# msyriac/orphics

Hardware: AMD Instinct MI355X
Metric: QE kappa reconstructions/sec on 8192^2 maps (higher is better)
Workload: dtype f64

## Files before the change

### orphics_amd/csrc/fft.hip

```cpp
#include <cmath>
#include <vector>
#include "fft_launch.hpp"
#include "fft_r2c_w64.hpp"
#include "fft_r2c_rs4096.hpp"
#include "fft_divbin.hpp"

namespace oa {

template <typename T, int MODE, class SEQ>
__global__ __launch_bounds__(row_maxnt<SEQ>(), waves_per_eu<T>()) void row_fft_kernel(RowArgs<T> a) {
    GpuCtx c{oa_dyn_smem};
    row_fft_body<T, MODE, SEQ>(c, a);
}

#ifndef OA_W64_OCC
#define OA_W64_OCC 1
#endif
__global__ __launch_bounds__(64, OA_W64_OCC) void row_r2c_w64_kernel(RowW64Args a) {
    GpuCtx c{oa_dyn_smem};
    row_r2c_w64_body(c, a);
}

template <typename T, class SEQ, int LR, bool PF>
__global__ __launch_bounds__(row_maxnt<SEQ>(), (sizeof(T) == 8 || PF ? 2 : 3)) void row_r2c_rsplit_kernel(RowArgs<T> a) {
// ... 28 lines not shown
    row_r2c_rs_body<T, 13, 3, PF>(c, a);
}

template <typename T, class SEQF, int LR, int LOGC>
__global__ __launch_bounds__((sizeof(T) == 8 ? 512 : 1024)) void col_fband_pack_kernel(ColFBandArgs<T> a, cx<T>* out) {
    GpuCtx c{nullptr};
    col_fband_pack_body<T, SEQF, LR, LOGC>(c, a, out);
}
template <typename T, class SEQF, int LR, int LOGC>
__global__ __launch_bounds__((sizeof(T) == 8 ? 512 : 1024), (sizeof(T) == 8 ? 2 : 4)) void col_fband_kernel(ColFBandArgs<T> a) {
    GpuCtx c{oa_dyn_smem};
    col_fband_body<T, SEQF, LR, LOGC>(c, a);
}

template <typename T, class SEQF, int LOGC>
__global__ __launch_bounds__((sizeof(T) == 8 ? 512 : 1024)) void col_fband3_pack_kernel(ColFBandArgs<T> a, cx<T>* out) {
    GpuCtx c{nullptr};
    col_fband3_pack_body<T, SEQF, LOGC>(c, a, out);
}
template <typename T, class SEQF, int LOGC>
__global__ __launch_bounds__((sizeof(T) == 8 ? 512 : 1024), (sizeof(T) == 8 ? 2 : 4)) void col_fband3_kernel(ColFBandArgs<T> a) {
    GpuCtx c{oa_dyn_smem};
    col_fband3_body<T, SEQF, LOGC>(c, a);
}

__global__ __launch_bounds__(128, 1) void row_r2c_w64x2_kernel(RowW64Args a) {
    GpuCtx c{oa_dyn_smem};
    row_r2c_w64x2_body(c, a);
}

#ifndef OA_QE_WAVES_PER_EU
#define OA_QE_WAVES_PER_EU 3
#endif
template <typename T, class SEQ> constexpr int qe_waves_per_eu() {
    return sizeof(T) == 8 ? 1 : (row_maxnt<SEQ>() > 256 ? 2 : OA_QE_WAVES_PER_EU);
}

template <typename T, class SEQ, int NZ>
__global__ __launch_bounds__(row_maxnt<SEQ>(), (qe_waves_per_eu<T, SEQ>())) void row_qe_kernel(RowQeArgs<T> a) {
    GpuCtx c{oa_dyn_smem};
#ifdef OA_QE_INPLACE
    row_qe_body_inplace<T, SEQ>(c, a);
#else
    row_qe_body<T, SEQ, NZ>(c, a);
#endif
}
// ... 260 lines not shown
            if (e != hipSuccess) rc = fail(std::string("fft launch: ") + hipGetErrorString(e));
        });
        if (!ok) rc = fail("fft: unsupported R-split column stage");
    }
    template <typename T>
    void col_fband3(int gx, int gz, size_t smem, int logMy, const ColFBandArgs<T>& a) {
        if (rc) return;
        constexpr int nt = sizeof(T) == 4 ? 1024 : 512, lc11 = sizeof(T) == 4 ? 3 : 2;
        if (logMy == 11) go(col_fband3_kernel<T, Seq<16, 16, 8>, lc11>, dim3(gx, 4, gz), nt, smem, a);
        else if (logMy == 10) go(col_fband3_kernel<T, Seq<16, 8, 8>, lc11 + 1>, dim3(gx, 4, gz), nt, smem, a);
        else rc = fail("fft: unsupported 3 x 2^k R-split column stage");
    }
    template <typename T>
    void col_fband3_pack(int gx, int logMy, const ColFBandArgs<T>& a, cx<T>* out) {
        if (rc) return;
        constexpr int nt = sizeof(T) == 4 ? 1024 : 512, lc11 = sizeof(T) == 4 ? 3 : 2;
        if (logMy == 11) hipLaunchKernelGGL((col_fband3_pack_kernel<T, Seq<16, 16, 8>, lc11>), dim3(gx, 4), dim3(nt), 0, st, a, out);
        else if (logMy == 10) hipLaunchKernelGGL((col_fband3_pack_kernel<T, Seq<16, 8, 8>, lc11 + 1>), dim3(gx, 4), dim3(nt), 0, st, a, out);
        else { rc = fail("fft: unsupported 3 x 2^k R-split column stage"); return; }
        const hipError_t e = hipGetLastError();
        if (e != hipSuccess) rc = fail(std::string("fft launch: ") + hipGetErrorString(e));
    }
    template <typename T>
    void row_qe(int grid, int nt, size_t smem, const RowQeArgs<T>& a) {
        const bool ok = dispatch_seq_qe(a.logL, [&](auto seq) {
            using S = decltype(seq);
            if constexpr (seq_logl<S>() >= 4) {
                if (nt > row_maxnt<S>()) { if (!rc) rc = fail("fft: row workgroup size exceeds its launch bound"); return; }
                if constexpr (S::n >= 2 && sizeof(T) == 4) {
                    dispatch_nz<S>(qe_first_stage_nz(a.logL, S::rget(0), a.win), [&](auto nzc) {
                        go(row_qe_kernel<T, S, decltype(nzc)::value>, dim3(grid), nt, smem, a);
                    });
                } else {
                    go(row_qe_kernel<T, S, 0>, dim3(grid), nt, smem, a);
                }
            } else {
                if (!rc) rc = fail("fft: unsupported row length");
            }
        });
        if (!ok && !rc) rc = fail("fft: unsupported row length");
    }
    template <typename T>
    void row_qe_pair8(int pairs, int M, const RowQeArgs<T>& a) {
        const bool ok = dispatch_rq8(M, a.win, a.lr, a.chain != nullptr, [&](auto ac, auto nzc, auto lay, auto ch) {
            constexpr int A = decltype(ac)::value;
            if (ch.value && !a.tab) { if (!rc) rc = fail("fft: estimator chains need a table"); return; }
// ... 748 lines not shown
```

### orphics_amd/csrc/fft_fband.hpp

```cpp
#pragma once
#include "fft_kernels.hpp"
#include "fft_mixed.hpp"
#ifndef FB_STAMP
#define FB_STAMP(i)
#endif

namespace oa {

template <typename T>
struct ColFBandArgs {
    const cx<T>* in;
    long kplane, pitch;
    const T* FG; const T* FH;
    long fpitch;
    const cx<T>* fgh;
    const T* lxd; const T* lyd;
    cx<T>* gx; cx<T>* gy; cx<T>* h;
    long opitch;
    int width;
    const cx<T>* tw;
    int ny_full, rband;
    long in_moff, out_moff;
    const cx<T>* tw3 = nullptr;
};
// ... 276 lines not shown
    const FBand3Store<T> st{outp + zmap * a.out_moff + (long)k1 * a.opitch + c0, (unsigned)(R * a.opitch), leg < 3 ? ncols : 0, ti, q};
    fft_pipeline<T, false, false, true, SI>(ctx, s + sid * (Q << LOGC), tq, NTS, logQ, LOGC, 0, twq, logQ, NoLoad{}, st);
    FB_STAMP(5);
}

template <typename T, class SEQF, int LOGC, class Ctx>
OA_HD void col_fband3_pack_body(Ctx& ctx, const ColFBandArgs<T>& a, cx<T>* out) {
    constexpr int logL = seq_total_log<SEQF>(), R = 4, Q = 1 << (logL - 4), C = 1 << LOGC;
    constexpr int NT = (1 << (logL + LOGC)) / EPT;
    const int tid = ctx.tid(), tile = ctx.bid_x(), k1 = ctx.bid_y(), c0 = tile << LOGC;
    const int c = tid & (C - 1), m = tid >> LOGC;
    cx<T>* o = out + (((long)k1 * ctx.grid_x() + tile) * 3) * NT + tid;
#pragma unroll
    for (int e = 0; e < 3; ++e) {
        const int yf = k1 + R * fband3_bin<Q>(m, e);
        bool live = c0 + c < a.width;
        if (a.rband) live = live && !(yf >= a.rband && yf <= a.ny_full - a.rband);
        cx<T> f = mk<T>((T)0, (T)0);
        if (live) { const long fi = (long)yf * a.fpitch + (c0 + c); f = mk<T>(a.FG[fi], a.FH[fi]); }
        o[e * NT] = f;
    }
}

}
```

### orphics_amd/csrc/fft_plan.hpp

```cpp
#pragma once
#include <cmath>
#include <cstdlib>
#include <vector>
#include "fft_kernels.hpp"
#include "fft_fband.hpp"
#include "fft_rowqe8.hpp"

namespace oa {

template <typename T>
inline std::vector<cx<T>> make_twiddles(int M) {
    std::vector<cx<T>> t((size_t)M);
    const long double tau = 6.283185307179586476925286766559005768L;
    for (int k = 0; k < M; ++k) {
        long double a = tau * (long double)k / (long double)M;
        t[(size_t)k].x = (T)cosl(a);
        t[(size_t)k].y = (T)(-sinl(a));
    }
    return t;
}

inline long kpitch_for(int nx) { return nx / 2 + 16; }

inline bool is_pow2(int v) { return v > 0 && (v & (v - 1)) == 0; }
inline bool is_m3(int v) { return v >= 3 && v % 3 == 0 && is_pow2(v / 3); }
// ... 75 lines not shown
        static const int narrow = [] { const char* e = exp_env("OA_FBAND_NARROW"); return e ? atoi(e) : 0; }();
        return (sizeof(T) == 4 ? 14 : 13) - (narrow > 0 ? 1 : 0);
    }
    template <class Launcher>
    void legs_fband(Launcher& q, const Fft2dPlan<T>& cv, const cx<T>* Y, long kplane, long pin, const T* FG, const T* FH, const T* lxd,
                    const T* lyd, cx<T>* gx, cx<T>* gy, cx<T>* h, int wmax, int rband, long pout, int nmaps = 1, long in_moff = 0,
                    long out_moff = 0, const cx<T>* fgh = nullptr, cx<T>* pack_out = nullptr) const {
        ColFBandArgs<T> a{};
        a.in = Y; a.kplane = kplane; a.pitch = pin; a.FG = FG; a.FH = FH; a.fpitch = kp; a.lxd = lxd; a.lyd = lyd; a.fgh = fgh;
        a.gx = gx; a.gy = gy; a.h = h; a.opitch = pout; a.width = clampw(wmax); a.tw = cv.tw_y; a.ny_full = ny; a.rband = clampr(rband);
        a.in_moff = in_moff; a.out_moff = out_moff;
        const int lt = fband_lt(), lc = lt - cv.logNy, Cs = 1 << lc;
        const int logMq = cv.logNy - (logNy - cv.logNy);
        const size_t smem = ((size_t)(1 << lt) + tw_lds_size(cv.logNy) + tw_lds_size(logMq) + (logNy - cv.logNy == 1 ? 0 : (1 << logMq))) * sizeof(cx<T>);
        if (pack_out) q.col_fband_pack((a.width + Cs - 1) / Cs, 1 << (logNy - cv.logNy), cv.logNy, a, pack_out);
        else q.col_fband((a.width + Cs - 1) / Cs, 1 << (logNy - cv.logNy), nmaps, smem, cv.logNy, a);
    }
    static bool has_rsplit3(int logNy, int logNx, int my3, int wl) {
        if (!is_m3(my3)) return false;
        const int myf = m3_pow2(my3);
        return (myf == 1024 || myf == 2048) && logNy - ilog2(myf) == 2 && has_rsplit(logNy, logNx, myf, wl) && fband_lt() == (sizeof(T) == 4 ? 14 : 13) &&
               div_lt() == fband_lt();
    }
    template <class Launcher>
    void legs_fband3(Launcher& q, const Fft2dPlan<T>& cv, const cx<T>* twf, const cx<T>* Y, long kplane, long pin, const T* FG, const T* FH,
                     const T* lxd, const T* lyd, cx<T>* gx, cx<T>* gy, cx<T>* h, int wmax, int rband, long pout, int nmaps = 1, long in_moff = 0,
                     long out_moff = 0, const cx<T>* fgh = nullptr, cx<T>* pack_out = nullptr) const {
        ColFBandArgs<T> a{};
        a.in = Y; a.kplane = kplane; a.pitch = pin; a.FG = FG; a.FH = FH; a.fpitch = kp; a.lxd = lxd; a.lyd = lyd; a.fgh = fgh;
        a.gx = gx; a.gy = gy; a.h = h; a.opitch = pout; a.width = clampw(wmax); a.tw = twf; a.tw3 = cv.tw_y; a.ny_full = ny; a.rband = clampr(rband);
        a.in_moff = in_moff; a.out_moff = out_moff;
        const int logMy = logNy - 2, lt = fband_lt(), lc = lt - logMy, Cs = 1 << lc, logQ = logMy - 4;
        const size_t smem = ((size_t)(1 << lt) + tw_lds_size(logMy) + tw_lds_size(logQ) + 3 * (1 << logQ)) * sizeof(cx<T>);
        if (pack_out) q.col_fband3_pack((a.width + Cs - 1) / Cs, logMy, a, pack_out);
        else q.col_fband3((a.width + Cs - 1) / Cs, nmaps, smem, logMy, a);
    }
    long fband_table_entries(const Fft2dPlan<T>& cv, int wmax) const {
        const int lc = fband_lt() - cv.logNy, Cs = 1 << lc;
        return (long)((clampw(wmax) + Cs - 1) / Cs) * Cs * cv.ny;
    }
    long fband3_table_entries(const Fft2dPlan<T>& cv, int wmax) const {
        const int lc = fband_lt() - (logNy - 2), Cs = 1 << lc;
        return (long)((clampw(wmax) + Cs - 1) / Cs) * Cs * cv.ny;
    }

    double row_grid_scale(int mrow) const { return (mrow > 0 && mrow < nx) ? (double)nx / (double)mrow : 1.0; }
    bool rows_qe_is_pair(int win, int wout, int mrow) const {
        if (mrow <= 0 || ny % 2) return false;
        const int M = mrow < nx ? mrow : nx;
        if (rq8_is_m3(M)) return rq8_ready(M) && rq8_covers(M, win, wout);
        return is_pow2(M) && M >= 1024 && M <= 8192 && 2L * win + wout <= M;
    }
    bool rows_qe_lr1(int win, int wout, int mrow) const { return mrow == 4096 && mrow <= nx && rq8_ready(mrow) && rq8_covers(mrow, win, wout); }
    static bool& rowqe8_on() {
        static bool on = exp_env("OA_NO_ROWQE8") == nullptr;
// ... 309 lines not shown
```

### orphics_amd/csrc/pipeline.hip

```cpp
#include <dlfcn.h>
#include <cstdlib>
#include <algorithm>
#include <string>
#include <utility>
#include <vector>
#include "common.hpp"
#include "fft_plan.hpp"

namespace oa {

constexpr int MC_BATCH_MAX = 6;

struct Pipeline {
    const void* FG = nullptr; const void* FH = nullptr; const void* Fn = nullptr;
    int wl = 0, wk = 0, rl = 0, rk = 0, mrow = -1;
    int mcol = -1;
    int my = 0;
    int my3 = 0;
    int map_grid() const { return my3 ? my3 : my; }
    void* work = nullptr;
    void* c[3] = {nullptr, nullptr, nullptr};
    void* g[2] = {nullptr, nullptr};
    void* kT = nullptr;
    void* kk = nullptr;
// ... 162 lines not shown
    q->my3 = 0;
    const bool want3 = q->mcol > 0 && is_m3(q->mcol);
    const long need = std::max(2L * q->rl + q->rk, 2L * q->rk);
    if (want3 && q->rl > 0 && q->rk > 0 && q->mcol < need)
        return fail("column grid < max(2*leg_rows + kappa_rows, 2*kappa_rows) would alias the leg products into the kept rows");
    if (int rc = resolve_my(p, q->mcol, q->rl, q->rk, &q->my)) return rc;
    const int my3 = want3 ? q->mcol : (q->mcol < 0 && q->my > 0 && q->my % 4 == 0 ? q->my / 4 * 3 : 0);
    bool ok = my3 > 0 && q->my == m3_pow2(my3) && my3 >= need && qe_rsplit_lr(p, q->my, q->wl, q->wk, q->mrow) == 2;
    if (ok) {
        if (int rc = plan_ensure_col_grid(p, my3)) return rc;
        ok = qe_rsplit_lr(p, my3, q->wl, q->wk, q->mrow) == 2;
    }
    if (ok) q->my3 = my3;
    else if (want3) return fail("oa_plan_set_col_grid: this geometry has no from-map path on a 3 x 2^k column grid (built for 8192-row maps on 1536 "
                                "rows and 4096-row maps on 768 rows, R-split from-map path)");
    return 0;
}

}

using namespace oa;

static int ensure_div_tables(oa_plan* p, oa::Pipeline* q, hipStream_t st);
static int ensure_div_tables(oa_plan* p, oa::Pipeline* q, hipStream_t st, int rows);
namespace oa {
static int band_grid_rule(const oa_plan* p, int mrow, int mcol, int wl, int wk, int rl, int rk, int* my, int* mx);
static int mixed_bind(oa_plan* p, Pipeline* q);
static int mixed_bins(oa_plan* p, Pipeline* q, hipStream_t st);
static int mixed_qe_tt(oa_plan* p, Pipeline* q, const void* map, const void* kX, const void* kY, void* out, int zero_outside, hipStream_t st);
static int mixed_moments(oa_plan* p, Pipeline* q, const void* map, int64_t* n, double* S, double* C, hipStream_t st);
static int mixed_mc_run(oa_plan* p, Pipeline* q, uint64_t base_seed, long sim_lo, long sim_hi, const void* covsqrt_hc, int64_t* n, double* S,
                        double* C, double* meanfield_acc, hipStream_t st);
static void band_options(Pipeline* q);
struct MvCall {
    int nest; const int* npieces; const double* signs; const void* const* FG; const void* const* FH; const int* swap;
    const void* const* kX; const void* const* kY; const void* const* Fn; bool pol;
    int nmaps; const void* const* maps; const void* rot_c; const void* rot_s; const int* xsrc; const int* ysrc;
};
static int mixed_qe_mv(oa_plan* p, Pipeline* q, const MvCall& c, void* out, int accumulate, int wl, int wk, int rl, int rk, int mrow, int zero_outside,
                       hipStream_t st);
static int mixed_qe_tt_splits(oa_plan* p, Pipeline* q, const char* who, int nsplits, const void* const* host_kmaps, void* const* host_out,
                              void* out_power, double norm, int zero_outside, hipStream_t st);
}
#define OA_NOT_MIXED(p, what) \
    OA_REQUIRE(!(p)->mixed, what ": not available on map sides that are not powers of two (one-call TT entries there: oa_qe_tt, oa_qe_tt_moments(2), oa_mc_run)")

extern "C" {

int oa_plan_set_col_grid(oa_plan* p, int mcol) {
    OA_REQUIRE(p, "oa_plan_set_col_grid: NULL plan");
    OA_REQUIRE(p->pow2 || p->mixed, "oa_plan_set_col_grid: map sides with a prime factor other than 2, 3 and 5 (chirp-z transforms) have no one-call path");
    OA_REQUIRE(mcol <= 0 || is_pow2(mcol) || (is_m3(mcol) && p->pow2),
               "oa_plan_set_col_grid: mcol must be -1 (auto), 0 (off), a power of two, or 3 x 2^k (from-map path of power-of-two plans)");
    Pipeline* q = pipe_of(p);
    q->mcol = mcol;
    if (p->mixed) {
        if (!q->FG) return 0;
        int my = 0, mx = 0;
        int rc = band_grid_rule(p, q->mrow, q->mcol, q->wl, q->wk, q->rl, q->rk, &my, &mx);
        if (!rc && q->band && my == q->bmy && mx == q->bmx) return 0;
        if (!rc) rc = mixed_bind(p, q);
        if (rc) q->FG = nullptr;
        return rc;
    }
    return q->FG ? resolve_col_grid(p, q) : 0;
}

int oa_plan_col_grid(const oa_plan* p) { return (p && p->pipe) ? ((Pipeline*)p->pipe)->map_grid() : 0; }

int oa_plan_band_grid(const oa_plan* p, int* my, int* mx) {
    OA_REQUIRE(p && my && mx, "oa_plan_band_grid: NULL argument");
    const Pipeline* q = (const Pipeline*)p->pipe;
    const bool bound = q && q->FG && q->band;
    *my = bound ? q->bmy : 0;
    *mx = bound ? q->bmx : 0;
    return 0;
}

int oa_plan_set_option(oa_plan* p, int option, int value) {
    OA_REQUIRE(p, "oa_plan_set_option: NULL plan");
    Pipeline* q = pipe_of(p);
    switch (option) {
        case OA_OPT_MC_BATCH:
            OA_REQUIRE(value >= 0 && value <= MC_BATCH_MAX, "oa_plan_set_option: OA_OPT_MC_BATCH takes 0 (default) .. 6");
            q->opt_mc_batch = value ? value : MC_BATCH_MAX; return 0;
        case OA_OPT_MV_BATCH: q->opt_mv_batch = value != 0; return 0;
        case OA_OPT_MV_ROWBATCH: q->opt_mv_rowbatch = value != 0; return 0;
        case OA_OPT_MV_CHAIN: q->opt_mv_chain = value != 0; return 0;
// ... 35 lines not shown

int oa_plan_set_filters(oa_plan* p, const void* FG, const void* FH, const void* Fnorm, int leg_cols, int kappa_cols,
                        int leg_rows, int kappa_rows, int mrow) {
    OA_REQUIRE(p && FG && FH && Fnorm, "oa_plan_set_filters: NULL argument");
    OA_REQUIRE(p->pow2 || p->mixed, "oa_plan_set_filters: map sides with a prime factor other than 2, 3 and 5 (chirp-z transforms) have no "
               "one-call path (use the modular oa_qe_legs / oa_mul_real / oa_qe_div calls)");
    OA_REQUIRE(p->have_laxes, "oa_plan_set_filters: call oa_plan_set_laxes first");
    if (p->pow2) {
        const int hw = p->nx / 2 + 1;
        OA_REQUIRE(leg_cols <= hw && kappa_cols <= hw, "oa_plan_set_filters: leg / kappa columns beyond the hc plane (> nx / 2 + 1)");
        OA_REQUIRE(2L * leg_rows - 1 <= p->ny && 2L * kappa_rows - 1 <= p->ny, "oa_plan_set_filters: leg / kappa rows beyond the plane (2 rows - 1 > ny)");
    }
    Pipeline* q = pipe_of(p);
    q->FG = FG; q->FH = FH; q->Fn = Fnorm;
    ++q->bind_gen;
    q->wl = leg_cols; q->wk = kappa_cols; q->rl = leg_rows; q->rk = kappa_rows; q->mrow = mrow;
    q->mcol = mrow == 0 ? 0 : -1;
    if (int rc = ensure_work(p, q)) { if (p->mixed) q->FG = nullptr; return rc; }
    if (p->mixed) {
        int rc = mixed_bind(p, q);
        if (rc) q->FG = nullptr;
        return rc;
    }
    return resolve_col_grid(p, q);
}

int oa_plan_set_bins(oa_plan* p, const int32_t* ids_hc, int nids, double norm, void* stream) {
    OA_REQUIRE(p && ids_hc && nids >= 3, "oa_plan_set_bins: bad argument");
    Pipeline* q = pipe_of(p);
    if (int rc = ensure_work(p, q)) return rc;
    if (q->nids != nids) {
        if (q->bin_scratch) { OA_HIP(hipDeviceSynchronize()); (void)hipFree(q->bin_scratch); (void)hipFree(q->sums); (void)hipFree(q->counts_full); (void)hipFree(q->counts_tmp); }
        const long sb = oa_bin_scratch_bytes(nids);
        OA_REQUIRE(sb > 0, "oa_plan_set_bins: bad nids");
        OA_HIP(hipMalloc(&q->bin_scratch, (size_t)sb * MC_BATCH_MAX));
        OA_HIP(hipMalloc((void**)&q->sums, MC_BATCH_MAX * nids * sizeof(double)));
        OA_HIP(hipMalloc((void**)&q->counts_full, nids * sizeof(int64_t)));
        OA_HIP(hipMalloc((void**)&q->counts_tmp, MC_BATCH_MAX * nids * sizeof(int64_t)));
    }
    if (!q->ticket) {
        OA_HIP(hipMalloc((void**)&q->ticket, sizeof(unsigned)));
        OA_HIP(hipMemset(q->ticket, 0, sizeof(unsigned)));
    }
    q->ids = ids_hc; q->nids = nids; q->norm = norm;
    ++q->bind_gen;
    if (int rc = oa_bin_power(p->dtype, q->c[0], q->c[0], norm, ids_hc, nullptr, (long)p->ny * p->kp, nids, p->kp, p->nx / 2, q->sums,
                              q->counts_full, nullptr, q->bin_scratch, 0, 0, stream)) return rc;
// ... 11 lines not shown
    const int logc = div_tile_logc(p, rows);
    if (t->tab_gen == q->bind_gen && t->tab_rows == rows && t->tab_logc == logc && t->tab_wk == q->wk) return 0;
    const size_t rs = p->dtype == OA_F32 ? 4 : 8;
    const long tiles = ((long)q->wk + (1 << logc) - 1) >> logc, total = (tiles * rows) << logc;
    if (t->fn_t_bytes < (size_t)total * rs) {
        if (t->fn_t) { OA_HIP(hipDeviceSynchronize()); (void)hipFree(t->fn_t); t->fn_t = nullptr; }
        OA_HIP(hipMalloc(&t->fn_t, (size_t)total * rs));
        t->fn_t_bytes = (size_t)total * rs;
    }
    if (t->ids_t_bytes < (size_t)total * 4) {
        if (t->ids_t) { OA_HIP(hipDeviceSynchronize()); (void)hipFree(t->ids_t); t->ids_t = nullptr; }
        OA_HIP(hipMalloc((void**)&t->ids_t, (size_t)total * 4));
        t->ids_t_bytes = (size_t)total * 4;
    }
    if (int rc = pack_tiles(p, q->Fn, t->fn_t, rows, logc, q->wk, (int)rs, st)) return rc;
    if (int rc = pack_tiles(p, q->ids, t->ids_t, rows, logc, q->wk, 4, st)) return rc;
    t->tab_gen = q->bind_gen; t->tab_rows = rows; t->tab_logc = logc; t->tab_wk = q->wk;
    return 0;
}
static int ensure_div_tables(oa_plan* p, Pipeline* q, hipStream_t st) {
    if (int rc = ensure_div_tables(p, q, st, q->my)) return rc;
    return q->my3 ? ensure_div_tables(p, q, st, q->my3) : 0;
}
static const void* fband_table(oa_plan* p, Pipeline* q, hipStream_t st) {
    static const bool off = exp_env("OA_NO_FBAND_TABLE") != nullptr;
    const int my = q->map_grid();
    if (off || !q->FG || my <= 0 || !qe_rsplit_lr(p, my, q->wl, q->wk, q->mrow)) return nullptr;
    if (q->fb_t && q->fb_gen == q->bind_gen && q->fb_my == my && q->fb_wl == q->wl && q->fb_rl == q->rl) return q->fb_t;
    const size_t need = (size_t)qe_fband_table_entries(p, q->wl, my) * 2 * (p->dtype == OA_F32 ? 4 : 8);
    if (q->fb_t_bytes < need) {
        if (q->fb_t) { if (hipDeviceSynchronize() != hipSuccess) return nullptr; (void)hipFree(q->fb_t); q->fb_t = nullptr; q->fb_t_bytes = 0; }
        if (hipMalloc(&q->fb_t, need) != hipSuccess) { q->fb_t = nullptr; (void)hipGetLastError(); return nullptr; }
        q->fb_t_bytes = need;
    }
    if (qe_fband_pack_w(p, q->FG, q->FH, q->fb_t, q->wl, q->rl, my, st)) return nullptr;
    q->fb_gen = q->bind_gen; q->fb_my = my; q->fb_wl = q->wl; q->fb_rl = q->rl;
    return q->fb_t;
}
static DivBinFuse make_fuse(const oa_plan* p, const Pipeline* q, int64_t* n, double* S, double* C, int store, int rows = -1) {
    DivBinFuse f{};
    if (rows < 0) rows = q->my;
    const Pipeline::DivTabs& t = q->tabs_of(rows);
    if (t.tab_rows && t.tab_gen == q->bind_gen && t.tab_rows == rows && t.tab_wk == q->wk) {
        f.ids_t = t.ids_t; f.fn_t = t.fn_t; f.tab_logc = t.tab_logc; f.tab_rows = t.tab_rows;
    }
    f.ids = q->ids; f.ipitch = p->kp; f.pnorm = q->norm; f.nids = q->nids; f.nxh = p->nx / 2;
    f.part = (double*)q->bin_scratch; f.part_cap = (long)(oa_bin_scratch_bytes(q->nids) / (long)sizeof(double)) * MC_BATCH_MAX;
    f.sums = q->sums; f.ticket = q->ticket; f.mcounts = q->counts_full; f.n = n; f.S = S; f.C = C; f.store = store; f.done = false;
    return f;
}

static int qe_tt_impl(oa_plan* p, const void* real_map, const void* kX, const void* kY, void* out_kappa_hc, int zero_outside,
                      void* stream, DivBinFuse* fuse, int rows_done = 0);
int oa_qe_tt(oa_plan* p, const void* real_map, const void* kX, const void* kY, void* out_kappa_hc, int zero_outside,
             void* stream) {
    if (p && p->mixed) {
        OA_REQUIRE(p->pipe && ((Pipeline*)p->pipe)->FG, "oa_qe_tt: call oa_plan_set_filters first");
        OA_REQUIRE((real_map != nullptr) != (kX != nullptr), "oa_qe_tt: pass either a real map or the Fourier-space leg(s)");
        return mixed_qe_tt(p, (Pipeline*)p->pipe, real_map, kX, kY, out_kappa_hc, zero_outside, (hipStream_t)stream);
    }
    return qe_tt_impl(p, real_map, kX, kY, out_kappa_hc, zero_outside, stream, nullptr);
}
static int qe_tt_impl(oa_plan* p, const void* real_map, const void* kX, const void* kY, void* out_kappa_hc, int zero_outside,
                      void* stream, DivBinFuse* fuse, int rows_done) {
    OA_REQUIRE(p && p->pipe && ((Pipeline*)p->pipe)->FG, "oa_qe_tt: call oa_plan_set_filters first");
    OA_REQUIRE((real_map != nullptr) != (kX != nullptr), "oa_qe_tt: pass either a real map or the Fourier-space leg(s)");
    Pipeline* q = (Pipeline*)p->pipe;
    void* out = out_kappa_hc ? out_kappa_hc : q->kk;
    if (out_kappa_hc && zero_outside)
        if (int rc = zero_complement(p, out, q->wk, q->rk, (hipStream_t)stream)) return rc;
    const long pl = work_pitch(p, q->wl), pk = work_pitch(p, q->wk);
    hipStream_t st = (hipStream_t)stream;
    int rc;
    const int my = (real_map && !rows_done) ? q->map_grid() : q->my;
    const int lr = (real_map && !rows_done) ? qe_rsplit_lr(p, my, q->wl, q->wk, q->mrow) : 0;
    if (real_map) rc = qe_map_legs_cols_w(p, real_map, q->FG, q->FH, q->c[0], q->c[1], q->c[2], q->wl, q->rl, pl, st, rows_done ? 6 : 7, my, lr,
                                          lr ? fband_table(p, q, st) : nullptr);
    else rc = qe_legs_cols_w(p, kX, kY ? kY : kX, q->FG, q->FH, q->c[0], q->c[1], q->c[2], q->wl, q->rl, pl, st, my);
    if (rc) return rc;
    const double s = 1.0 / ((double)p->ny * p->nx), sy = my ? (double)p->ny / my : 1.0;
    if ((rc = qe_rows_w(p, q->c[0], q->c[1], q->c[2], q->g[0], q->g[1], s * s * sy, 0, q->wl, q->wk, q->mrow, pl, pk, st, my, lr))) return rc;
    return qe_cols_div_w(p, q->g[0], q->g[1], q->Fn, out, 0, q->wk, q->rk, pk, st, my, fuse);
}

int oa_qe_pol(oa_plan* p, int npieces, const double* host_signs, const void* const* host_FG, const void* const* host_FH,
              const int* host_swap, const void* kX, const void* kY, const void* Fnorm, void* out, int accumulate,
              int leg_cols, int kappa_cols, int leg_rows, int kappa_rows, int mrow, int zero_outside, void* stream) {
    OA_REQUIRE(p && npieces >= 1 && host_signs && host_FG && host_FH && kX && kY && Fnorm && out, "oa_qe_pol: bad argument");
    OA_REQUIRE(p->pow2 || p->mixed, "oa_qe_pol: map sides with a prime factor other than 2, 3 and 5 (chirp-z transforms) have no one-call path "
               "(use the modular oa_qe_legs / oa_mul_real / oa_qe_div calls)");
    Pipeline* q = pipe_of(p);
    if (p->mixed) {
        const MvCall c{1, &npieces, host_signs, host_FG, host_FH, host_swap, &kX, &kY, &Fnorm, true};
        return mixed_qe_mv(p, q, c, out, accumulate, leg_cols, kappa_cols, leg_rows, kappa_rows, mrow, zero_outside, (hipStream_t)stream);
    }
    if (int rc = ensure_work(p, q)) return rc;
    if (!accumulate && zero_outside && out != q->kk)
        if (int rc = zero_complement(p, out, kappa_cols, kappa_rows, (hipStream_t)stream)) return rc;
    const long pl = work_pitch(p, leg_cols), pk = work_pitch(p, kappa_cols);
    hipStream_t st = (hipStream_t)stream;
// ... 354 lines not shown
    return 0;
}

int oa_qe_tt_split_power(oa_plan* p, int nsplits, const void* const* host_kmaps, void* out_hcreal, double norm, int zero_outside, void* stream) {
    OA_REQUIRE(p && host_kmaps && out_hcreal, "oa_qe_tt_split_power: bad argument");
    OA_REQUIRE(nsplits >= 4 && nsplits <= 8, "oa_qe_tt_split_power: 4 <= nsplits <= 8");
    OA_REQUIRE(!p->pow2, "oa_qe_tt_split_power: a power-of-two plan has no band grid; there the estimate is oa_qe_tt_splits + oa_split_cross_power");
    OA_REQUIRE(p->pipe && ((Pipeline*)p->pipe)->FG, "oa_qe_tt_split_power: call oa_plan_set_filters first");
    return mixed_qe_tt_splits(p, (Pipeline*)p->pipe, "oa_qe_tt_split_power", nsplits, host_kmaps, nullptr, out_hcreal, norm, zero_outside,
                              (hipStream_t)stream);
}

int oa_qe_tt_moments2(oa_plan* p, const void* real_map0, const void* real_map1, int64_t* n, double* S, double* C, void* stream) {
    OA_REQUIRE(p && p->pipe && ((Pipeline*)p->pipe)->FG && ((Pipeline*)p->pipe)->ids, "oa_qe_tt_moments2: call oa_plan_set_filters and oa_plan_set_bins first");
    OA_REQUIRE(real_map0 && real_map1 && n && S && C, "oa_qe_tt_moments2: NULL argument");
    Pipeline* q = (Pipeline*)p->pipe;
    if (p->mixed) {
        if (int rc = mixed_moments(p, q, real_map0, n, S, C, (hipStream_t)stream)) return rc;
        return mixed_moments(p, q, real_map1, n, S, C, (hipStream_t)stream);
    }
    const long pl = work_pitch(p, q->wl), pk = work_pitch(p, q->wk);
    if (int rc = ensure_div_tables(p, q, (hipStream_t)stream)) return rc;
    DivBinFuse f = make_fuse(p, q, n, S, C, 0, q->map_grid());
    int rc = qe_tt_pair_w(p, real_map0, real_map1, q->FG, q->FH, q->Fn, q->c[0], q->c[1], q->c[2], q->g[0], q->g[1], q->kk, q->kT, q->wl,
                          q->wk, q->rl, q->rk, q->mrow, q->map_grid(), pl, pk, (hipStream_t)stream, divbin_enabled(q) ? &f : nullptr,
                          fband_table(p, q, (hipStream_t)stream));
    if (rc > 0) return rc;
    if (rc == 0 && f.done) return 0;
    if (rc < 0) {
        if ((rc = oa_qe_tt_moments(p, real_map0, n, S, C, stream))) return rc;
        return oa_qe_tt_moments(p, real_map1, n, S, C, stream);
    }
    const long es = 2 * (p->dtype == OA_F32 ? 4 : 8);
    const long back = ((const char*)q->kT - (const char*)q->kk) / es;
    return bin_power_moments(p->dtype, q->kk, q->norm, q->ids, (long)p->ny * p->kp, q->nids, p->kp, p->nx / 2, q->sums, q->counts_tmp,
                             q->bin_scratch, q->wk, q->rk, q->ticket, q->counts_full, n, S, C, (hipStream_t)stream, 2, back);
}

int oa_qe_tt_stage(oa_plan* p, int stage, const void* real_map, void* stream) {
    OA_REQUIRE(p && p->pipe && ((Pipeline*)p->pipe)->FG, "oa_qe_tt_stage: call oa_plan_set_filters first");
    OA_NOT_MIXED(p, "oa_qe_tt_stage");
    Pipeline* q = (Pipeline*)p->pipe;
    const long pl = work_pitch(p, q->wl), pk = work_pitch(p, q->wk);
    hipStream_t st = (hipStream_t)stream;
    const int my = q->map_grid();
    const double s = 1.0 / ((double)p->ny * p->nx), sy = my ? (double)p->ny / my : 1.0;
    const int lr = qe_rsplit_lr(p, my, q->wl, q->wk, q->mrow);
    switch (stage) {
        case 0: case 1: case 2:
            OA_REQUIRE(real_map, "oa_qe_tt_stage: stages 0-2 need the map");
            return qe_map_legs_cols_w(p, real_map, q->FG, q->FH, q->c[0], q->c[1], q->c[2], q->wl, q->rl, pl, st, 1 << stage, my, lr,
                                      lr ? fband_table(p, q, st) : nullptr);
        case 3: return qe_rows_w(p, q->c[0], q->c[1], q->c[2], q->g[0], q->g[1], s * s * sy, 0, q->wl, q->wk, q->mrow, pl, pk, st, my, lr);
        case 4: {
            if (q->ids && divbin_enabled(q)) {
                DivBinFuse f = make_fuse(p, q, (int64_t*)q->kT, (double*)q->kT + 8, (double*)q->kT + 8 + q->nids, 0, my);
                return qe_cols_div_w(p, q->g[0], q->g[1], q->Fn, q->kk, 0, q->wk, q->rk, pk, st, my, &f);
            }
            return qe_cols_div_w(p, q->g[0], q->g[1], q->Fn, q->kk, 0, q->wk, q->rk, pk, st, my);
        }
        case 5: {
            OA_REQUIRE(q->ids, "oa_qe_tt_stage: stage 5 needs oa_plan_set_bins");
            if (oa_plan_div_fused(p)) return 0;
            int64_t* n = (int64_t*)q->kT;
            double* S = (double*)q->kT + 8;
            double* C = S + q->nids;
            return bandpower_moments(p, q, n, S, C, stream);
        }
        default: return fail("oa_qe_tt_stage: stage must be 0..5");
    }
}

}

namespace oa {
// ... 585 lines not shown
```

Before: 5933.

## Add streamed f64 R-split column kernel and presize filter table at bind time

Adds a new 256-thread column stage for the 3x2^k R-split path. It streams the 8 input decimation phases per wave, accumulating into registers and combining in LDS, so it avoids holding a full-column tile in LDS. The default enables it for f64 when the radial band fits. This aims for higher occupancy and smaller LDS use in exchange for more twiddle multiplies and extra syncs. Separately, the packed filter table is now allocated when filters or the grid are set, which removes the hipDeviceSynchronize/hipMalloc from the hot path and makes missing sizing an error.

```diff
diff --git a/orphics_amd/csrc/fft.hip b/orphics_amd/csrc/fft.hip
--- a/orphics_amd/csrc/fft.hip
+++ b/orphics_amd/csrc/fft.hip
@@ -74,6 +74,17 @@
 __global__ __launch_bounds__((sizeof(T) == 8 ? 512 : 1024), (sizeof(T) == 8 ? 2 : 4)) void col_fband3_kernel(ColFBandArgs<T> a) {
     GpuCtx c{oa_dyn_smem};
     col_fband3_body<T, SEQF, LOGC>(c, a);
+}
+
+template <typename T, int LOGMY, int LOGC>
+__global__ __launch_bounds__(256) void col_fband3s_pack_kernel(ColFBandArgs<T> a, cx<T>* out) {
+    GpuCtx c{nullptr};
+    col_fband3s_pack_body<T, LOGMY, LOGC>(c, a, out);
+}
+template <typename T, int LOGMY, int LOGC>
+__global__ __launch_bounds__(256, 2) void col_fband3s_kernel(ColFBandArgs<T> a) {
+    GpuCtx c{oa_dyn_smem};
+    col_fband3s_body<T, LOGMY, LOGC>(c, a);
 }
 
 __global__ __launch_bounds__(128, 1) void row_r2c_w64x2_kernel(RowW64Args a) {
@@ -380,6 +391,27 @@
         if (e != hipSuccess) rc = fail(std::string("fft launch: ") + hipGetErrorString(e));
     }
     template <typename T>
+    void col_fband3s(int gx, int gz, size_t smem, int logMy, const ColFBandArgs<T>& a) {
+        if (rc) return;
+        constexpr int nt = 256;
+        if (smem > 78 * 1024) { rc = fail("fft: the streamed R-split column stage takes at most 78 KB of LDS"); return; }
+        if constexpr (Fft2dPlan<T>::fband3_stream_default()) {
+            if (logMy == 11) { go(col_fband3s_kernel<T, 11, 2>, dim3(gx, 4, gz), nt, smem, a); return; }
+            if (logMy == 10) { go(col_fband3s_kernel<T, 10, 3>, dim3(gx, 4, gz), nt, smem, a); return; }
+        }
+        rc = fail("fft: unsupported 3 x 2^k R-split column stage");
+    }
+    template <typename T>
+    void col_fband3s_pack(int gx, int logMy, const ColFBandArgs<T>& a, cx<T>* out) {
+        if (rc) return;
+        constexpr int nt = 256;
+        if (Fft2dPlan<T>::fband3_stream_default() && logMy == 11) hipLaunchKernelGGL((col_fband3s_pack_kernel<T, 11, 2>), dim3(gx, 4), dim3(nt), 0, st, a, out);
+        else if (Fft2dPlan<T>::fband3_stream_default() && logMy == 10) hipLaunchKernelGGL((col_fband3s_pack_kernel<T, 10, 3>), dim3(gx, 4), dim3(nt), 0, st, a, out);
+        else { rc = fail("fft: unsupported 3 x 2^k R-split column stage"); return; }
+        const hipError_t e = hipGetLastError();
+        if (e != hipSuccess) rc = fail(std::string("fft launch: ") + hipGetErrorString(e));
+    }
+    template <typename T>
     void row_qe(int grid, int nt, size_t smem, const RowQeArgs<T>& a) {
         const bool ok = dispatch_seq_qe(a.logL, [&](auto seq) {
             using S = decltype(seq);
diff --git a/orphics_amd/csrc/fft_fband.hpp b/orphics_amd/csrc/fft_fband.hpp
--- a/orphics_amd/csrc/fft_fband.hpp
+++ b/orphics_amd/csrc/fft_fband.hpp
@@ -322,4 +322,182 @@
     }
 }
 
-}
+template <int Q>
+OA_HD int fband3s_bin(int m, int e) { return e ? 15 * Q + m : m; }
+
+template <typename T, int LOGMY, int LOGC, class Ctx>
+OA_HD void col_fband3s_body(Ctx& ctx, const ColFBandArgs<T>& a) {
+    cx<T>* s = reinterpret_cast<cx<T>*>(ctx.smem());
+    constexpr int R = 4, D = 8;
+    constexpr int My = 1 << LOGMY, logQ = LOGMY - 4, Q = 1 << logQ, Mq = 3 * Q;
+    constexpr int LOGP = LOGMY - 3, P = 1 << LOGP, R2 = P / 16, NB2 = EPT / R2;
+    constexpr int C = 1 << LOGC, NW = 4, NT = 64 * NW;
+    constexpr int NTS = (Q << LOGC) / EPT;
+    static_assert(P * C == 64 * EPT && 2 * NT == Q * C && 8 * NTS == NT && (R2 == 8 || R2 == 16), "col_fband3s: geometry");
+    const int tid = ctx.tid();
+    int tile = ctx.bid_x();
+    if ((sizeof(cx<T>) << LOGC) < 128) {
+        constexpr int G = 128 / (int)(sizeof(cx<T>) << LOGC), GW = 8 * G;
+        const int nt = ctx.grid_x(), base = tile & ~(GW - 1), r = tile & (GW - 1);
+        if (base + GW <= nt) tile = base + G * (r & 7) + (r >> 3);
+    }
+    const int c0 = tile << LOGC;
+    const int k1 = ctx.bid_y();
+    int ncols = a.width - c0;
+    if (ncols > C) ncols = C;
+    cx<T>* twl = s + 1024 * NW;
+    cx<T>* twp = twl + tw_lds_size(LOGMY);
+    cx<T>* twq = twp + tw_lds_size(LOGP);
+    cx<T>* ti = twq + tw_lds_size(logQ);
+    tw_lds_fill<T>(ctx, twl, a.tw, LOGMY, LOGMY, NT);
+    tw_lds_fill<T>(ctx, twp, a.tw, LOGMY, LOGP, NT);
+    tw_lds_fill<T>(ctx, twq, a.tw, LOGMY, logQ, NT);
+    for (int i = tid; i < Mq; i += NT) ti[i] = a.tw3[(unsigned)k1 * (unsigned)i];
+    ctx.sync();
+    const long zmap = ctx.bid_z();
+    {
+        const int w = tid >> 6, lane = tid & 63;
+        cx<T>* sw = s + 1024 * w;
+        cx<T> acc[EPT];
+#pragma unroll
+        for (int i = 0; i < EPT; ++i) acc[i] = mk<T>((T)0, (T)0);
+        const cx<T>* in0 = a.in + zmap * a.in_moff + (long)k1 * a.kplane + c0;
+        cx<T> v[EPT], vn[EPT];
+        stage_in<T, 16, false, true>(sw, v, lane, 64, LOGP, LOGC, 0, 0, twp, LOGP, ColLoad<T>{in0 + (long)w * a.pitch, (unsigned)(D * a.pitch), ncols, false});
+        stage_out<T, 16, false, false>(sw, v, lane, 64, LOGP, LOGC, 0, 0, NoStore{});
+        {
+            const ColLoad<T> ldn{in0 + (long)(w + 4) * a.pitch, (unsigned)(D * a.pitch), ncols, false};
+#pragma unroll
+            for (int t = 0; t < 16; ++t) vn[t] = ldn.template get<T>((lane >> LOGC) + (t << (LOGP - 4)), lane & (C - 1));
+        }
+#pragma unroll 1
+        for (int r = w; r < D; r += 4) {
+            if (r >= 4) {
+                Dft<T, 16>::run(vn);
+                ctx.wsync();
+                stage_out<T, 16, false, false>(sw, vn, lane, 64, LOGP, LOGC, 0, 0, NoStore{});
+            }
+            ctx.wsync();
+            stage_in<T, R2, false, false>(sw, v, lane, 64, LOGP, LOGC, 0, 4, twp, LOGP, NoLoad{});
+#pragma unroll
+            for (int u = 0; u < NB2; ++u) {
+                const int j = (lane + u * 64) >> LOGC;
+#pragma unroll
+                for (int t = 0; t < R2; ++t) {
+                    const int kap = j + 16 * t, ks = kap < P / 2 ? kap : kap - P;
+                    acc[u * R2 + t] = acc[u * R2 + t] + v[u * R2 + t] * tw_lds(twl, tw_lds_h(LOGMY), (r * ks) & (My - 1));
+                }
+            }
+        }
+        ctx.wsync();
+#pragma unroll
+        for (int u = 0; u < NB2; ++u) {
+            const int b = lane + u * 64, cw = b & (C - 1), j = b >> LOGC;
+#pragma unroll
+            for (int t = 0; t < R2; ++t) sw[((j + 16 * t) << LOGC) + cw] = acc[u * R2 + t];
+        }
+    }
+    const int c = tid & (C - 1), m0 = tid >> LOGC;
+    const bool ok = c < ncols;
+    T fgv[4], fhv[4], lyv[4];
+    bool lv[4];
+    cx<T> wq1[2], wq2[2];
+    const cx<T>* fq = a.fgh ? a.fgh + (((long)k1 * ctx.grid_x() + tile) * 4) * NT + tid : nullptr;
+    const T lx = ldg(a.lxd + (ok ? c0 + c : 0));
+#pragma unroll
+    for (int p = 0; p < 2; ++p) {
+        const int m = m0 + p * (Q / 2);
+        wq1[p] = ldg(a.tw3 + 4 * m); wq2[p] = ldg(a.tw3 + 8 * m);
+#pragma unroll
+        for (int e = 0; e < 2; ++e) {
+            const int yf = k1 + R * fband3s_bin<Q>(m, e);
+            const bool live = ok && !(yf >= a.rband && yf <= a.ny_full - a.rband);
+            if (fq) {
+                const cx<T> f = ldg(fq + (2 * p + e) * NT);
+                fgv[2 * p + e] = f.x; fhv[2 * p + e] = f.y;
+            } else {
+                const long fi = live ? (long)yf * a.fpitch + (c0 + c) : 0;
+                fgv[2 * p + e] = ldg(a.FG + fi);
+                fhv[2 * p + e] = ldg(a.FH + fi);
+            }
+            lyv[2 * p + e] = ldg(a.lyd + (live ? yf : 0));
+            lv[2 * p + e] = live;
+        }
+    }
+    ctx.sync();
+    cx<T> xv[4];
+    {
+        const cx<T>* sg = s + c;
+#pragma unroll
+        for (int p = 0; p < 2; ++p)
+#pragma unroll
+            for (int e = 0; e < 2; ++e) {
+                const int at = (m0 + p * (Q / 2) + e * Q) << LOGC;
+                xv[2 * p + e] = ((sg[at] + sg[1024 + at]) + sg[2048 + at]) + sg[3072 + at];
+            }
+    }
+    ctx.sync();
+    cx<T> gyv[6];
+#pragma unroll
+    for (int p = 0; p < 2; ++p) {
+        const int m = m0 + p * (Q / 2);
+        cx<T> zh[3], zx[3], zy[3];
+        zh[1] = zx[1] = zy[1] = mk<T>((T)0, (T)0);
+#pragma unroll
+        for (int e = 0; e < 2; ++e) {
+            const int i = 2 * p + e;
+            const cx<T> x = xv[i];
+            const T fg = lv[i] ? fgv[i] : (T)0, fh = lv[i] ? fhv[i] : (T)0, ly = lv[i] ? lyv[i] : (T)0;
+            const cx<T> g = mul_pi(x * fg);
+            zh[2 * e] = swp(x * fh);
+            zx[2 * e] = swp(g * (ok ? lx : (T)0));
+            zy[2 * e] = swp(g * ly);
+        }
+        MrDft<T, 3>::run(zh); MrDft<T, 3>::run(zx); MrDft<T, 3>::run(zy);
+#pragma unroll
+        for (int q = 0; q < 3; ++q) {
+            const int at = ((q * Q + m) << LOGC) + c;
+            cx<T> h = zh[q], x = zx[q], y = zy[q];
+            if (q == 1) { h = h * wq1[p]; x = x * wq1[p]; y = y * wq1[p]; }
+            if (q == 2) { h = h * wq2[p]; x = x * wq2[p]; y = y * wq2[p]; }
+            s[at] = h;
+            s[(Mq << LOGC) + at] = x;
+            gyv[3 * p + q] = y;
+        }
+    }
+    ctx.sync();
+    const int sid = tid / NTS, tq = tid - sid * NTS;
+    const int leg = sid / 3, q = sid - 3 * leg;
+    using SI = typename SeqOf<logQ>::type;
+    const long ooff = zmap * a.out_moff + (long)k1 * a.opitch + c0;
+    const FBand3Store<T> st{(leg == 0 ? a.h : a.gx) + ooff, (unsigned)(R * a.opitch), leg < 2 ? ncols : 0, ti, q};
+    fft_pipeline<T, false, false, true, SI>(ctx, s + sid * (Q << LOGC), tq, NTS, logQ, LOGC, 0, twq, logQ, NoLoad{}, st);
+    ctx.sync();
+#pragma unroll
+    for (int p = 0; p < 2; ++p)
+#pragma unroll
+        for (int qq = 0; qq < 3; ++qq) s[((qq * Q + m0 + p * (Q / 2)) << LOGC) + c] = gyv[3 * p + qq];
+    ctx.sync();
+    const FBand3Store<T> st2{a.gy + ooff, (unsigned)(R * a.opitch), leg == 0 ? ncols : 0, ti, q};
+    fft_pipeline<T, false, false, true, SI>(ctx, s + sid * (Q << LOGC), tq, NTS, logQ, LOGC, 0, twq, logQ, NoLoad{}, st2);
+}
+
+template <typename T, int LOGMY, int LOGC, class Ctx>
+OA_HD void col_fband3s_pack_body(Ctx& ctx, const ColFBandArgs<T>& a, cx<T>* out) {
+    constexpr int R = 4, Q = 1 << (LOGMY - 4), C = 1 << LOGC, NT = (Q * C) / 2;
+    const int tid = ctx.tid(), tile = ctx.bid_x(), k1 = ctx.bid_y(), c0 = tile << LOGC;
+    const int c = tid & (C - 1), m0 = tid >> LOGC;
+    cx<T>* o = out + (((long)k1 * ctx.grid_x() + tile) * 4) * NT + tid;
+#pragma unroll
+    for (int p = 0; p < 2; ++p)
+#pragma unroll
+        for (int e = 0; e < 2; ++e) {
+            const int yf = k1 + R * fband3s_bin<Q>(m0 + p * (Q / 2), e);
+            const bool live = c0 + c < a.width && !(yf >= a.rband && yf <= a.ny_full - a.rband);
+            cx<T> f = mk<T>((T)0, (T)0);
+            if (live) { const long fi = (long)yf * a.fpitch + (c0 + c); f = mk<T>(a.FG[fi], a.FH[fi]); }
+            o[(2 * p + e) * NT] = f;
+        }
+}
+
+}
diff --git a/orphics_amd/csrc/fft_plan.hpp b/orphics_amd/csrc/fft_plan.hpp
--- a/orphics_amd/csrc/fft_plan.hpp
+++ b/orphics_amd/csrc/fft_plan.hpp
@@ -1,6 +1,8 @@
 #pragma once
 #include <cmath>
 #include <cstdlib>
+#include <type_traits>
+#include <utility>
 #include <vector>
 #include "fft_kernels.hpp"
 #include "fft_fband.hpp"
@@ -122,15 +124,29 @@
         return (myf == 1024 || myf == 2048) && logNy - ilog2(myf) == 2 && has_rsplit(logNy, logNx, myf, wl) && fband_lt() == (sizeof(T) == 4 ? 14 : 13) &&
                div_lt() == fband_lt();
     }
+    static bool fband3_streams(int logMy, int rband) { return rband > 0 && 2 * ((rband + 3) / 4) <= (1 << (logMy - 3)); }
+    static constexpr bool fband3_stream_default() { return sizeof(T) == 8; }
+    template <class L, class = void> struct has_fband3s : std::false_type {};
+    template <class L>
+    struct has_fband3s<L, std::void_t<decltype(std::declval<L&>().col_fband3s(0, 0, (size_t)0, 0, std::declval<const ColFBandArgs<T>&>()))>> : std::true_type {};
     template <class Launcher>
     void legs_fband3(Launcher& q, const Fft2dPlan<T>& cv, const cx<T>* twf, const cx<T>* Y, long kplane, long pin, const T* FG, const T* FH,
                      const T* lxd, const T* lyd, cx<T>* gx, cx<T>* gy, cx<T>* h, int wmax, int rband, long pout, int nmaps = 1, long in_moff = 0,
-                     long out_moff = 0, const cx<T>* fgh = nullptr, cx<T>* pack_out = nullptr) const {
+                     long out_moff = 0, const cx<T>* fgh = nullptr, cx<T>* pack_out = nullptr, int body = -1) const {
         ColFBandArgs<T> a{};
         a.in = Y; a.kplane = kplane; a.pitch = pin; a.FG = FG; a.FH = FH; a.fpitch = kp; a.lxd = lxd; a.lyd = lyd; a.fgh = fgh;
         a.gx = gx; a.gy = gy; a.h = h; a.opitch = pout; a.width = clampw(wmax); a.tw = twf; a.tw3 = cv.tw_y; a.ny_full = ny; a.rband = clampr(rband);
         a.in_moff = in_moff; a.out_moff = out_moff;
         const int logMy = logNy - 2, lt = fband_lt(), lc = lt - logMy, Cs = 1 << lc, logQ = logMy - 4;
+        if constexpr (has_fband3s<Launcher>::value) {
+            if ((body < 0 ? fband3_stream_default() : body > 0) && fband3_streams(logMy, a.rband)) {
+                const int Ct = 1 << (13 - logMy);
+                const size_t smem3 = ((size_t)4096 + tw_lds_size(logMy) + tw_lds_size(logMy - 3) + tw_lds_size(logQ) + 3 * (1 << logQ)) * sizeof(cx<T>);
+                if (pack_out) q.col_fband3s_pack((a.width + Ct - 1) / Ct, logMy, a, pack_out);
+                else q.col_fband3s((a.width + Ct - 1) / Ct, nmaps, smem3, logMy, a);
+                return;
+            }
+        }
         const size_t smem = ((size_t)(1 << lt) + tw_lds_size(logMy) + tw_lds_size(logQ) + 3 * (1 << logQ)) * sizeof(cx<T>);
         if (pack_out) q.col_fband3_pack((a.width + Cs - 1) / Cs, logMy, a, pack_out);
         else q.col_fband3((a.width + Cs - 1) / Cs, nmaps, smem, logMy, a);
diff --git a/orphics_amd/csrc/pipeline.hip b/orphics_amd/csrc/pipeline.hip
--- a/orphics_amd/csrc/pipeline.hip
+++ b/orphics_amd/csrc/pipeline.hip
@@ -208,6 +208,7 @@
 using namespace oa;
 
 static int ensure_div_tables(oa_plan* p, oa::Pipeline* q, hipStream_t st);
+static int fband_table_size(oa_plan* p, oa::Pipeline* q);
 static int ensure_div_tables(oa_plan* p, oa::Pipeline* q, hipStream_t st, int rows);
 namespace oa {
 static int band_grid_rule(const oa_plan* p, int mrow, int mcol, int wl, int wk, int rl, int rk, int* my, int* mx);
@@ -249,7 +250,9 @@
         if (rc) q->FG = nullptr;
         return rc;
     }
-    return q->FG ? resolve_col_grid(p, q) : 0;
+    if (!q->FG) return 0;
+    if (int rc = resolve_col_grid(p, q)) return rc;
+    return fband_table_size(p, q);
 }
 
 int oa_plan_col_grid(const oa_plan* p) { return (p && p->pipe) ? ((Pipeline*)p->pipe)->map_grid() : 0; }
@@ -331,7 +334,8 @@
         if (rc) q->FG = nullptr;
         return rc;
     }
-    return resolve_col_grid(p, q);
+    if (int rc = resolve_col_grid(p, q)) return rc;
+    return fband_table_size(p, q);
 }
 
 int oa_plan_set_bins(oa_plan* p, const int32_t* ids_hc, int nids, double norm, void* stream) {
@@ -389,20 +393,32 @@
     if (int rc = ensure_div_tables(p, q, st, q->my)) return rc;
     return q->my3 ? ensure_div_tables(p, q, st, q->my3) : 0;
 }
-static const void* fband_table(oa_plan* p, Pipeline* q, hipStream_t st) {
+static bool fband_table_wanted(const oa_plan* p, const Pipeline* q, int my) {
     static const bool off = exp_env("OA_NO_FBAND_TABLE") != nullptr;
+    return !off && q->FG && my > 0 && qe_rsplit_lr(p, my, q->wl, q->wk, q->mrow);
+}
+static int fband_table_size(oa_plan* p, Pipeline* q) {
     const int my = q->map_grid();
-    if (off || !q->FG || my <= 0 || !qe_rsplit_lr(p, my, q->wl, q->wk, q->mrow)) return nullptr;
-    if (q->fb_t && q->fb_gen == q->bind_gen && q->fb_my == my && q->fb_wl == q->wl && q->fb_rl == q->rl) return q->fb_t;
+    if (!fband_table_wanted(p, q, my)) return 0;
     const size_t need = (size_t)qe_fband_table_entries(p, q->wl, my) * 2 * (p->dtype == OA_F32 ? 4 : 8);
-    if (q->fb_t_bytes < need) {
-        if (q->fb_t) { if (hipDeviceSynchronize() != hipSuccess) return nullptr; (void)hipFree(q->fb_t); q->fb_t = nullptr; q->fb_t_bytes = 0; }
-        if (hipMalloc(&q->fb_t, need) != hipSuccess) { q->fb_t = nullptr; (void)hipGetLastError(); return nullptr; }
-        q->fb_t_bytes = need;
-    }
-    if (qe_fband_pack_w(p, q->FG, q->FH, q->fb_t, q->wl, q->rl, my, st)) return nullptr;
-    q->fb_gen = q->bind_gen; q->fb_my = my; q->fb_wl = q->wl; q->fb_rl = q->rl;
-    return q->fb_t;
+    if (q->fb_t_bytes >= need) return 0;
+    if (q->fb_t) { OA_HIP(hipDeviceSynchronize()); (void)hipFree(q->fb_t); q->fb_t = nullptr; q->fb_t_bytes = 0; q->fb_gen = 0; }
+    OA_HIP(hipMalloc(&q->fb_t, need));
+    q->fb_t_bytes = need;
+    return 0;
+}
+static int fband_table(oa_plan* p, Pipeline* q, hipStream_t st, const void** tab) {
+    *tab = nullptr;
+    const int my = q->map_grid();
+    if (!fband_table_wanted(p, q, my)) return 0;
+    if (q->fb_gen != q->bind_gen || q->fb_my != my || q->fb_wl != q->wl || q->fb_rl != q->rl) {
+        const size_t need = (size_t)qe_fband_table_entries(p, q->wl, my) * 2 * (p->dtype == OA_F32 ? 4 : 8);
+        if (!q->fb_t || q->fb_t_bytes < need) return fail("R-split column stage: the packed filter table was not sized for this binding (oa_plan_set_filters)");
+        if (int rc = qe_fband_pack_w(p, q->FG, q->FH, q->fb_t, q->wl, q->rl, my, st)) return rc;
+        q->fb_gen = q->bind_gen; q->fb_my = my; q->fb_wl = q->wl; q->fb_rl = q->rl;
+    }
+    *tab = q->fb_t;
+    return 0;
 }
 static DivBinFuse make_fuse(const oa_plan* p, const Pipeline* q, int64_t* n, double* S, double* C, int store, int rows = -1) {
     DivBinFuse f{};
@@ -441,8 +457,9 @@
     int rc;
     const int my = (real_map && !rows_done) ? q->map_grid() : q->my;
     const int lr = (real_map && !rows_done) ? qe_rsplit_lr(p, my, q->wl, q->wk, q->mrow) : 0;
-    if (real_map) rc = qe_map_legs_cols_w(p, real_map, q->FG, q->FH, q->c[0], q->c[1], q->c[2], q->wl, q->rl, pl, st, rows_done ? 6 : 7, my, lr,
-                                          lr ? fband_table(p, q, st) : nullptr);
+    const void* fgh = nullptr;
+    if (real_map && lr) if ((rc = fband_table(p, q, st, &fgh))) return rc;
+    if (real_map) rc = qe_map_legs_cols_w(p, real_map, q->FG, q->FH, q->c[0], q->c[1], q->c[2], q->wl, q->rl, pl, st, rows_done ? 6 : 7, my, lr, fgh);
     else rc = qe_legs_cols_w(p, kX, kY ? kY : kX, q->FG, q->FH, q->c[0], q->c[1], q->c[2], q->wl, q->rl, pl, st, my);
     if (rc) return rc;
     const double s = 1.0 / ((double)p->ny * p->nx), sy = my ? (double)p->ny / my : 1.0;
@@ -843,9 +860,10 @@
     const long pl = work_pitch(p, q->wl), pk = work_pitch(p, q->wk);
     if (int rc = ensure_div_tables(p, q, (hipStream_t)stream)) return rc;
     DivBinFuse f = make_fuse(p, q, n, S, C, 0, q->map_grid());
+    const void* fgh = nullptr;
+    if (int rc = fband_table(p, q, (hipStream_t)stream, &fgh)) return rc;
     int rc = qe_tt_pair_w(p, real_map0, real_map1, q->FG, q->FH, q->Fn, q->c[0], q->c[1], q->c[2], q->g[0], q->g[1], q->kk, q->kT, q->wl,
-                          q->wk, q->rl, q->rk, q->mrow, q->map_grid(), pl, pk, (hipStream_t)stream, divbin_enabled(q) ? &f : nullptr,
-                          fband_table(p, q, (hipStream_t)stream));
+                          q->wk, q->rl, q->rk, q->mrow, q->map_grid(), pl, pk, (hipStream_t)stream, divbin_enabled(q) ? &f : nullptr, fgh);
     if (rc > 0) return rc;
     if (rc == 0 && f.done) return 0;
     if (rc < 0) {
@@ -868,10 +886,12 @@
     const double s = 1.0 / ((double)p->ny * p->nx), sy = my ? (double)p->ny / my : 1.0;
     const int lr = qe_rsplit_lr(p, my, q->wl, q->wk, q->mrow);
     switch (stage) {
-        case 0: case 1: case 2:
+        case 0: case 1: case 2: {
             OA_REQUIRE(real_map, "oa_qe_tt_stage: stages 0-2 need the map");
-            return qe_map_legs_cols_w(p, real_map, q->FG, q->FH, q->c[0], q->c[1], q->c[2], q->wl, q->rl, pl, st, 1 << stage, my, lr,
-                                      lr ? fband_table(p, q, st) : nullptr);
+            const void* fgh = nullptr;
+            if (lr) if (int rc = fband_table(p, q, st, &fgh)) return rc;
+            return qe_map_legs_cols_w(p, real_map, q->FG, q->FH, q->c[0], q->c[1], q->c[2], q->wl, q->rl, pl, st, 1 << stage, my, lr, fgh);
+        }
         case 3: return qe_rows_w(p, q->c[0], q->c[1], q->c[2], q->g[0], q->g[1], s * s * sy, 0, q->wl, q->wk, q->mrow, pl, pk, st, my, lr);
         case 4: {
             if (q->ids && divbin_enabled(q)) {
```

Result: slower. 5813 (-2.0%).
